# nrontsis/PILCO

Measured on AMD Instinct MI355X. Metric: moment-matching rollouts/sec (N=1000,D=10,E=10,H=40), higher is better.
Workload: dtype f64; 1 GPU; BASELINE configs[1]: N=1000 D=10 E=10 H=40 full rollout + reward, control_dim=0 (D==E read literally), ExponentialReward(W=I,t=0), factorisation cached (R-fwd); one step = one host-synchronised pilco_rollout call (what PILCO.predict makes) with its result downloaded; parallelism=pairs1, exchange=none (one rank)

## Files before the change

pilco_amd/csrc/glue_device.h:

```cpp
#pragma once
#include "mm_device.h"
#include "link_predicates.h"

namespace pilco {

struct GlueLds {
    double* mx;
    double* sx;
    double* mu;
    double* su;
    double* cxu;
    double* t1;
    double* t2;
    double* s1;
    double* jm;
    double* js;
    double* seg;
    double* mp;
    double* misc;
    double* pol;
    double* xm;
    double* xs;
    int nm;
    int o_sx, o_s1, o_js, o_seg, o_mp, o_misc;
};

__host__ __device__ __forceinline__ void glue_lds_carve(const GlueArgs& g, double* sm, GlueLds& L) {
    const int E = g.E, D = g.D;
    const int nm = E > D ? E : D;
    int seg_n = (g.flags & (GF_PACK | GF_ASSEMBLE)) ? g.wk.SEG * ((g.flags & GF_PACK) ? 1 : g.wk.nranks) : 0;
    if (g.flags & GF_RBF_POST) seg_n = g.pwk.SEG;
    L.mx = sm;
    L.sx = L.mx + nm;
    L.mu = L.sx + nm * nm;
    L.su = L.mu + nm;
    L.cxu = L.su + nm * nm;
    L.t1 = L.cxu + nm * nm;
    L.t2 = L.t1 + nm * nm;
    L.s1 = L.t2 + nm * nm;
    L.jm = L.s1 + nm * nm;
    L.js = L.jm + nm;
    L.misc = L.js + nm * nm;
    L.seg = L.misc + 256;
    L.mp = L.seg + seg_n;
    {
        const int mp_n = (g.flags & GF_RBF_POST) ? g.pwk.EL * g.pwk.NCHM * (1 + E) : ((g.flags & GF_PACK) ? g.wk.EL * g.wk.NCHM * (1 + D) : 0);
        const int rew_n = (int)reward_lds_doubles(E);
        const int tail = seg_n + mp_n;
        L.pol = L.seg + (tail > rew_n ? tail : rew_n);
    }
    L.xm = nullptr;
    L.xs = nullptr;
    L.nm = nm;
    L.o_sx = nm;
    L.o_s1 = 2 * nm + 5 * nm * nm;
    L.o_js = 3 * nm + 6 * nm * nm;
    L.o_seg = 3 * nm + 7 * nm * nm + 256;
    L.o_misc = 3 * nm + 7 * nm * nm;
    L.o_mp = L.o_seg + seg_n;
}

struct LoadSeg {
    int dst;
    const double* src;
    int n;
};
template <int NSEG, int MAXV>
__device__ __forceinline__ void multi_load(double* lds, const LoadSeg (&sg)[NSEG]) {
    int off[NSEG + 1];
    off[0] = 0;
#pragma unroll
    for (int i = 0; i < NSEG; ++i) off[i + 1] = off[i] + sg[i].n;
    const int total = off[NSEG];
    const int nthr = (int)blockDim.x;
    for (int base = 0; base < total; base += MAXV * nthr) {
        double v[MAXV];
#pragma unroll
        for (int k = 0; k < MAXV; ++k) {
            const int e = base + k * nthr + (int)threadIdx.x;
            v[k] = 0.0;
            if (e < total) {
#pragma unroll
                for (int i = 0; i < NSEG; ++i)
                    if (e >= off[i] && e < off[i + 1]) v[k] = sg[i].src[e - off[i]];
            }
        }
#pragma unroll
        for (int k = 0; k < MAXV; ++k) {
            const int e = base + k * nthr + (int)threadIdx.x;
            if (e < total) {
#pragma unroll
                for (int i = 0; i < NSEG; ++i)
                    if (e >= off[i] && e < off[i + 1]) lds[sg[i].dst + (e - off[i])] = v[k];
            }
        }
    }
}

__device__ __forceinline__ void squash_inplace(const GlueLds& L, int U, const double* maxact, double* cdiag, double* sc_alt = nullptr, bool eval_only = false) {
    const int t = threadIdx.x;
    const int nm = L.nm;
    double* sc = sc_alt ? sc_alt : L.t1;
    const int cap = sc_alt ? 5 * (U * U + U) : PILCO_SQUASH_ROUND_CAP(nm);
    const int nitems = U * U + U;
    double newS[4] = {0.0, 0.0, 0.0, 0.0};
    double newM = 0.0, newC = 0.0;
    for (int i0 = 0; i0 < 5 * nitems; i0 += cap) {
        const int n = (5 * nitems - i0) < cap ? (5 * nitems - i0) : cap;
        {
            const int w = t >> 6, f = w % 3, nw = (int)blockDim.x >> 6;
            const int nwf = (nw - f + 2) / 3;
            const int qa = i0 / 5, qb = (i0 + n) / 5;
            const int nc = (U * U > qa) ? ((U * U < qb ? U * U : qb) - qa) : 0, nu = (qb - qa) - nc;
            const int cnt = (f == 0) ? 3 * nc + nu : (f == 1) ? 2 * nc + nu : nu;
            for (int e = (w / 3) * 64 + (t & 63); e < cnt; e += nwf * 64) {
                int q, j;
                if (f == 0) {
                    if (e < 3 * nc) { q = qa + e / 3; j = e - 3 * (e / 3); } else { q = qa + nc + (e - 3 * nc); j = 0; }
                } else if (f == 1) {
                    if (e < 2 * nc) { q = qa + (e >> 1); j = 3 + (e & 1); } else { q = qa + nc + (e - 2 * nc); j = 1; }
                } else {
                    q = qa + nc + e; j = 2;
                }
                double arg;
                if (q < U * U) {
                    int v;
                    const int u = idiv_s(q, U, v);
                    const double lq = -(L.su[u * U + u] + L.su[v * U + v]) / 2.0;
                    const double suv = L.su[q];
                    arg = (j == 0) ? lq : (j == 1) ? lq + suv : (j == 2) ? lq - suv : (j == 3) ? L.mu[u] - L.mu[v] : L.mu[u] + L.mu[v];
                } else {
                    const int u = q - U * U;
                    arg = (j == 0) ? -L.su[u * U + u] / 2.0 : L.mu[u];
                }
                double val;
                if (f == 0) val = exp(arg);
                else if (f == 1) val = cos(arg);
                else val = sin(arg);
                sc[5 * (q - qa) + j] = val;
            }
        }
        __syncthreads();
        if (eval_only) return;
        const int q0 = i0 / 5, q1 = (i0 + n) / 5;
#pragma unroll
        for (int k = 0; k < 4; ++k) {
            const int e = t + k * (int)blockDim.x;
            if (e < U * U && e >= q0 && e < q1) {
                int v;
// ... 71 lines not shown
}

__device__ __forceinline__ void write_joint_lin_squash(const GlueArgs& g, const GlueLds& L, bool writer, const double* sq, const double* maxact) {
    const int E = g.E, U = g.U, D = g.D, t = threadIdx.x;
    double* s1_dst = g.s1_out ? g.s1_out : g.s1;
    auto cdiag_of = [&](int u) { const double* r = sq + 5 * (U * U + u); return (maxact ? maxact[u] : 1.0) * r[0] * r[1]; };
    if (t < D) {
        double v;
        if (t < E) v = L.mx[t];
        else {
            const int u = t - E;
            const double* r = sq + 5 * (U * U + u);
            v = (maxact ? maxact[u] : 1.0) * r[0] * r[2];
        }
        L.jm[t] = v;
        if (L.xm) L.xm[t] = v;
        if (writer) {
            g.wk.in_m[t] = v;
            if (g.tape) g.tape[(long)g.step * (D + D * D + E * D + E + E * E + D * E) + t] = v;
        }
    }
    for (int e = t; e < D * D; e += blockDim.x) {
        int c;
        const int r = idiv_s(e, D, c);
        double v;
        if (r < E && c < E) v = L.sx[r * E + c];
        else if (r < E) v = L.t1[(c - E) * E + r] * cdiag_of(c - E);
        else if (c < E) v = L.t1[(r - E) * E + c] * cdiag_of(r - E);
        else {
            const int u = r - E, v2 = c - E;
            const double* q = sq + 5 * (u * U + v2);
            const double val = (q[1] - q[0]) * q[3] - (q[2] - q[0]) * q[4];
            v = (maxact ? maxact[u] * maxact[v2] : 1.0) * val / 2.0;
        }
        L.js[e] = v;
        if (L.xs) L.xs[e] = v;
        if (writer) {
            g.wk.in_s[e] = v;
            if (r < E) s1_dst[r * D + c] = v;
            if (g.tape) {
                double* rec = g.tape + (long)g.step * (D + D * D + E * D + E + E * E + D * E);
                rec[D + e] = v;
                if (r < E) rec[D + D * D + r * D + c] = v;
            }
        }
    }
    __syncthreads();
}

struct PackPre {
    double v[16];
    double isdet;
};
__device__ __forceinline__ void mm_pack_issue(const MMWork& wk, int base, PackPre& pp) {
    const int t = threadIdx.x;
    const int k = base + (t >> 2), gq = t & 3;
    pp.isdet = 0.0;
#pragma unroll
    for (int u = 0; u < 16; ++u) pp.v[u] = 0.0;
    if (t >= 256 || k >= wk.PL) return;
    pp.isdet = wk.pair_isdet[k];
    if (wk.sk_waves > 0) {
        const int qw = wk.sk_maxw >> 2;
        const double* src = wk.sk_part + (long)(gq * qw) * wk.sk_pls + k;
#pragma unroll
        for (int u = 0; u < 16; ++u)
            if (u < qw) pp.v[u] = src[(long)u * wk.sk_pls];
    } else {
        const double* part = wk.pair_part + (long)k * wk.NT * 2;
        const int q0 = (int)((long)wk.NT * gq / 4), q1 = (int)((long)wk.NT * (gq + 1) / 4);
#pragma unroll
        for (int u = 0; u < 8; ++u)
            if (q0 + u < q1) {
                pp.v[2 * u] = part[2 * (q0 + u)];
                pp.v[2 * u + 1] = part[2 * (q0 + u) + 1];
            }
    }
}
__device__ __forceinline__ void mm_pack_sum(const MMWork& wk, int base, const PackPre& pp, double& s0, double& s1) {
    const int t = threadIdx.x;
    const int k = base + (t >> 2), gq = t & 3;
    s0 = 0.0;
    s1 = 0.0;
    if (t >= 256 || k >= wk.PL) return;
    if (wk.sk_waves > 0) {
#pragma unroll
        for (int u = 0; u < 16; ++u) s0 += pp.v[u];
        const int qw = wk.sk_maxw >> 2;
        const double* src = wk.sk_part + (long)(gq * qw) * wk.sk_pls + k;
        for (int u0 = 16; u0 < qw; u0 += 8) {
            double w8[8];
#pragma unroll
            for (int u = 0; u < 8; ++u) w8[u] = src[(long)min(u0 + u, qw - 1) * wk.sk_pls];
#pragma unroll
            for (int u = 0; u < 8; ++u) s0 += (u0 + u < qw) ? w8[u] : 0.0;
        }
    } else {
        const double* part = wk.pair_part + (long)k * wk.NT * 2;
        const int q0 = (int)((long)wk.NT * gq / 4), q1 = (int)((long)wk.NT * (gq + 1) / 4);
#pragma unroll
        for (int u = 0; u < 8; ++u)
            if (q0 + u < q1) {
                s0 += pp.v[2 * u];
                s1 += pp.v[2 * u + 1];
            }
        for (int q = q0 + 8; q < q1; ++q) {
            s0 += part[2 * q];
            s1 += part[2 * q + 1];
        }
    }
}

__device__ __forceinline__ void mm_pack(const MMWork& wk, int D, int E, const GlueLds& L, PackPre& pp, bool writer) {
    const int t = threadIdx.x;
    double* seg = wk.gath + (long)wk.rank * wk.SEG;
    for (int base = 0; base < wk.PL; base += 64) {
        const int k = base + (t >> 2), gq = t & 3;
        if (base > 0) mm_pack_issue(wk, base, pp);
        double s0, s1;
        mm_pack_sum(wk, base, pp, s0, s1);
        s0 += __shfl_xor(s0, 1);
        s1 += __shfl_xor(s1, 1);
        s0 += __shfl_xor(s0, 2);
        s1 += __shfl_xor(s1, 2);
        if (t < 256 && k < wk.PL && gq == 0) {
            const bool diag = k * wk.nranks + wk.rank < E;
            const double v = (diag ? (s0 - s1) : s0) * pp.isdet;
            if (writer) seg[k] = v;
            L.seg[k] = v;
        }
    }
    const int W1 = 1 + D;
    for (int e = t; e < wk.EL * W1; e += blockDim.x) {
        int idx;
        const int o = idiv_s(e, W1, idx);
        double sum = 0.0;
        _Pragma("unroll 8") for (int ch = 0; ch < wk.NCHM; ++ch) sum += L.mp[(o * wk.NCHM + ch) * W1 + idx];
        if (writer) seg[wk.OUTOFF + e] = sum;
        L.seg[wk.OUTOFF + e] = sum;
    }
    __syncthreads();
}

__device__ __forceinline__ void mm_assemble(const MMWork& wk, const double* src, const double* var, int D, int E, double* oM,
                            double* oS, double* oV, bool writer) {
    const int t = threadIdx.x;
    for (int a = t; a < E; a += blockDim.x) {
        const double v = src[(a % wk.nranks) * wk.SEG + wk.OUTOFF + (a / wk.nranks) * (1 + D)];
        oM[a] = v;
        if (writer) wk.out_M[a] = v;
    }
    for (int e = t; e < D * E; e += blockDim.x) {
        int a;
        const int d = idiv_s(e, E, a);
        const double v = src[(a % wk.nranks) * wk.SEG + wk.OUTOFF + (a / wk.nranks) * (1 + D) + 1 + d];
        oV[e] = v;
        if (writer) wk.out_V[e] = v;
    }
    __syncthreads();
    for (int e = t; e < E * E; e += blockDim.x) {
        int b;
        const int a = idiv_s(e, E, b);
        const int hi = a > b ? a : b, lo = a > b ? b : a;
        const int kk = pair_order_index(E, hi, lo);
        double v = src[(kk % wk.nranks) * wk.SEG + kk / wk.nranks];
        if (a == b) v += var[a];
        v = fma(-oM[a], oM[b], v);
        oS[e] = v;
        if (writer) wk.out_S[e] = v;
    }
    __syncthreads();
// ... 227 lines not shown
                        for (int c = 0; c < E; ++c) y = fma(Q[r * E + c], xrow[c], y);
                        quad = fma(xrow[r], y, quad);
                    }
                    vv[ii] = kk + quad;
                } else {
                    double* ytmp = pt + bf * (2 * E + 2) + ii * 16;
                    for (int r = 0; r < E; ++r) {
                        double y = 0.0;
                        for (int c = 0; c < E; ++c) y = fma(Q[r * E + c], xrow[c], y);
                        quad = fma(xrow[r], y, quad);
                        ytmp[r] = 2.0 * y;
                    }
                    for (int r = 0; r < E; ++r) xrow[r] = ytmp[r];
                    uv[ii] = kk + quad;
                }
            }
        }
        __syncthreads();
        if (do2 && t <= E) red[t] = ((red[t] + red[(E + 2) + t]) + red[2 * (E + 2) + t]) + red[3 * (E + 2) + t];
        if (do3 && t < 256) {
            double acc = 0.0;
            for (int idx = t; idx < bf * bf; idx += 256) {
                int j;
                const int i = idiv_s(idx, bf, j);
                double e = uv[i] + vv[j];
                for (int d = 0; d < E; ++d) e = fma(pv[i * E + d], wv[j * E + d], e);
                acc = fma(bet[a * bf + i] * bet[b * bf + j], exp(e), acc);
            }
            const double sacc = wave_sum_lane63(acc);
            if (lane == 63) red3[w] = sacc;
        }
        __syncthreads();
        if (do2) {
            const double cu = var[u] / sqrt(det[u]);
            if (t == 0) L.mu[u] = cu * red[0];
            if (t < E) {
                double acc = 0.0;
                for (int kq = 0; kq < E; ++kq) acc = fma(Tm[(u * E + t) * E + kq], red[1 + kq], acc);
                L.cxu[t * U + u] = cu * acc;
            }
        }
        if (do3 && t == 0) {
            const double N = (red3[0] + red3[1]) + (red3[2] + red3[3]);
            double v = N / sqrt(det[U + pq]);
            if (a == b) v += var[a];
            v = fma(-L.mu[a], L.mu[b], v);
            L.su[a * U + b] = v;
            L.su[b * U + a] = v;
        }
        __syncthreads();
    }
}

template <int PK = -1, bool SR = false>
__device__ __forceinline__ void glue_body(const GlueArgs& g, const GlueLds& L, bool writer) {
    const int E = g.E, D = g.D, U = g.U, t = threadIdx.x;
    int mp_n = (g.flags & GF_PACK) ? g.wk.EL * g.wk.NCHM * (1 + D) : 0;
    int seg_n = (g.flags & (GF_PACK | GF_ASSEMBLE)) ? g.wk.SEG * ((g.flags & GF_PACK) ? 1 : g.wk.nranks) : 0;
    if (g.flags & GF_RBF_POST) {
        mp_n = g.pwk.EL * g.pwk.NCHM * (1 + E);
        seg_n = g.pwk.SEG;
    }
    const bool dbg0 = (t == 0) && writer;
    const int dbo = g.dbg_off ? g.dbg_off : ((g.step == 0) ? 16 : 0);
    DBG_STAMP(g.wk, 8 + dbo, dbg0);
    PackPre pp;
    if ((g.flags & GF_PACK) && !MM_ABL(g.wk, 16)) mm_pack_issue(g.wk, 0, pp);
    const bool xq_in = !SR && g.xq && (g.flags & GF_ASSEMBLE) && !(g.flags & GF_PACK);
    if constexpr (!SR)
        if (xq_in) xq_wait(g);
    {
        const bool need_state = (g.flags & (GF_PROPAGATE | GF_TRAJ | GF_POLICY | GF_RBF_PRE)) != 0;
        const bool lin = (g.flags & GF_POLICY) && g.pol_kind == PILCO_POLICY_LINEAR;
        const bool pol = (g.flags & GF_POLICY) && g.pol_kind != PILCO_POLICY_NONE;
        const LoadSeg sg[8] = {
            {0, g.m_x, need_state ? E : 0},
            {L.o_sx, g.s_x, need_state ? E * E : 0},
            {L.o_s1, g.s1, (g.flags & GF_PROPAGATE) ? E * D : 0},
            {L.o_mp, (g.flags & GF_RBF_POST) ? g.pwk.mean_part : g.wk.mean_part, mp_n},
            {L.o_seg, g.wk.gath, ((g.flags & GF_ASSEMBLE) && !(g.flags & GF_PACK) && !xq_in) ? seg_n : 0},
            {L.o_js, g.W, lin ? U * E : 0},
            {L.o_misc + 128, g.b, lin ? U : 0},
            {L.o_misc + 160, g.maxact, (pol && g.maxact) ? U : 0},
        };
        RbfPre rpre;
        const bool rbf_in = (PK < 0 || PK == 2) && (g.flags & GF_POLICY) && g.pol_kind == PILCO_POLICY_RBF && g.pol_inline;
        if constexpr (PK < 0 || PK == 2)
            if (rbf_in) rbf_policy_preload_round(g, L, 0, rpre, true, false);
        multi_load<8, 4>(L.mx, sg);
        if constexpr (PK < 0 || PK == 2)
            if (rbf_in) rbf_policy_preload_rest(g, L, rpre);
        if constexpr (!SR)
            if (xq_in) xq_load_segments(g, L.seg);
    }
    __syncthreads();

    DBG_STAMP(g.wk, 9 + dbo, dbg0);
    if ((g.flags & GF_PACK) && !MM_ABL(g.wk, 16)) mm_pack(g.wk, D, E, L, pp, writer);
    if constexpr (!SR)
        if ((g.flags & GF_PACK) && g.xq_peers && writer) xq_push(g, L.seg);
    DBG_STAMP(g.wk, 10 + dbo, dbg0);
    const bool fast = (g.flags & (GF_PACK | GF_ASSEMBLE | GF_PROPAGATE)) == (GF_PACK | GF_ASSEMBLE | GF_PROPAGATE) && g.wk.nranks == 1;
    const bool joint_is_state = (PK == 0) && fast && (g.flags & GF_POLICY) && !g.act_out && U == 0;
    if (fast) {
        const double* seg = L.seg;
        const int W1 = 1 + D, OO = g.wk.OUTOFF;
        for (int e = t; e < E * E; e += blockDim.x) {
            int c;
            const int r = idiv_s(e, E, c);
            const int hi = r > c ? r : c, lo = r > c ? c : r;
            double v = seg[pair_order_index(E, hi, lo)];
            if (r == c) v += g.var[r];
            v = fma(-seg[OO + r * W1], seg[OO + c * W1], v);
            L.su[e] = v;
            double acc = 0.0;
            _Pragma("unroll 8") for (int k = 0; k < D; ++k) acc = fma(L.s1[r * D + k], seg[OO + c * W1 + 1 + k], acc);
            L.t1[e] = acc;
        }
        if (t < E) L.mu[t] = seg[OO + t * W1];
        if (writer && g.tape) {
            for (int e = t; e < D * E; e += blockDim.x) {
                int a_;
                const int d_ = idiv_s(e, E, a_);
                L.cxu[e] = seg[OO + a_ * W1 + 1 + d_];
            }
        }
        __syncthreads();
        if (writer && g.tape && g.step >= 1) {
            double* rec = g.tape + (long)(g.step - 1) * (D + D * D + E * D + E + E * E + D * E) + D + D * D + E * D;
            if (t < E) rec[t] = L.mu[t];
            for (int e = t; e < E * E; e += blockDim.x) rec[E + e] = L.su[e];
            for (int e = t; e < D * E; e += blockDim.x) rec[E + E * E + e] = L.cxu[e];
        }
        double* s1_dst = g.s1_out ? g.s1_out : g.s1;
        double* trec = g.tape ? g.tape + (long)g.step * (D + D * D + E * D + E + E * E + D * E) : nullptr;
        for (int e = t; e < E * E; e += blockDim.x) {
            int c;
            const int r = idiv_s(e, E, c);
            const double v = ((L.su[e] + L.sx[e]) + L.t1[e]) + L.t1[c * E + r];
            L.sx[e] = v;
            if (writer) g.s_out[e] = v;
            if (joint_is_state) {
                L.js[e] = v;
                if (L.xs) L.xs[e] = v;
                if (writer) {
                    g.wk.in_s[e] = v;
                    s1_dst[e] = v;
                    if (trec) {
                        trec[D + e] = v;
                        trec[D + D * D + e] = v;
                    }
// ... 25 lines not shown
        }
    }
    DBG_STAMP(g.wk, 11 + dbo, dbg0);
    if (!SR && !fast && (g.flags & GF_PROPAGATE)) {
        for (int e = t; e < E * E; e += blockDim.x) {
            int c;
            const int r = idiv_s(e, E, c);
            double acc = 0.0;
            _Pragma("unroll 8") for (int k = 0; k < D; ++k) acc = fma(L.s1[r * D + k], L.cxu[k * E + c], acc);
            L.t1[e] = acc;
        }
        __syncthreads();
        for (int e = t; e < E * E; e += blockDim.x) {
            int c;
            const int r = idiv_s(e, E, c);
            const double v = ((L.su[e] + L.sx[e]) + L.t1[e]) + L.t1[c * E + r];
            L.t2[e] = v;
            if (writer) g.s_out[e] = v;
        }
        if (t < E) {
            const double v = L.mu[t] + L.mx[t];
            L.misc[96 + t] = v;
            if (writer) g.m_out[t] = v;
        }
        __syncthreads();
        for (int e = t; e < E * E; e += blockDim.x) L.sx[e] = L.t2[e];
        if (t < E) L.mx[t] = L.misc[96 + t];
        __syncthreads();
    }
    DBG_STAMP(g.wk, 12 + dbo, dbg0);
    if (writer && (g.flags & GF_TRAJ) && g.traj) {
        double* dst = g.traj + (long)g.step * (E + E * E);
        if (t < E) dst[t] = L.mx[t];
        for (int e = t; e < E * E; e += blockDim.x) dst[E + e] = L.sx[e];
    }
    if (writer && (g.flags & GF_RBF_PRE)) {
        if (t < E) g.pwk.in_m[t] = L.mx[t];
        for (int e = t; e < E * E; e += blockDim.x) g.pwk.in_s[e] = L.sx[e];
    }
    if (g.flags & GF_POLICY) {
        const double* jcd = nullptr;
        bool lin_fused = false;
        if (PK != 0 && PK != 3 && g.pol_kind == PILCO_POLICY_RBF) {
            bool done = false;
            if constexpr (PK < 0 || PK == 2) {
                if (g.pol_inline) {
                    rbf_policy_inline(g, L);
                    done = true;
                }
            }
            if constexpr (PK < 0 || PK == 1) {
                if (!done) {
                    PackPre pq;
                    mm_pack_issue(g.pwk, 0, pq);
                    mm_pack(g.pwk, E, U, L, pq, writer);
                    mm_assemble(g.pwk, L.seg, g.pvar, E, U, L.mu, L.su, L.cxu, writer);
                }
            }
            if (t < U) L.su[t * U + t] -= g.pvar[t] - 1e-6;
            __syncthreads();
            if (g.squash) {
                double* cdiag = L.misc + 1;
                squash_inplace(L, U, g.maxact ? L.misc + 160 : nullptr, cdiag);
                if (g.act_out) {
                    for (int e = t; e < E * U; e += blockDim.x) L.cxu[e] *= cdiag[e % U];
                    __syncthreads();
                } else {
                    jcd = cdiag;
                }
            }
        }
        if ((PK < 0 || PK == 3) && g.pol_kind == PILCO_POLICY_LINEAR) {
            if (t < U) {
                double acc = L.misc[128 + t];
                _Pragma("unroll 8") for (int k = 0; k < E; ++k) acc = fma(L.js[t * E + k], L.mx[k], acc);
                L.mu[t] = acc;
            }
            for (int e = t; e < U * E; e += blockDim.x) {
                int c;
                const int u = idiv_s(e, E, c);
                double acc = 0.0;
                _Pragma("unroll 8") for (int k = 0; k < E; ++k) acc = fma(L.js[u * E + k], L.sx[k * E + c], acc);
                L.t1[e] = acc;
                L.cxu[c * U + u] = L.js[e];
            }
            __syncthreads();
            for (int e = t; e < U * U; e += blockDim.x) {
                int v;
                const int u = idiv_s(e, U, v);
                double acc = 0.0;
                _Pragma("unroll 8") for (int k = 0; k < E; ++k) acc = fma(L.t1[u * E + k], L.js[v * E + k], acc);
                L.su[e] = acc;
            }
            __syncthreads();
#ifdef LINK_STAMPS
            DBG_STAMP(g.wk, 36, dbg0);
#endif
            if (g.squash) {
                double* cdiag = L.misc + 1;
                lin_fused = !g.act_out && !joint_is_state && PILCO_SQUASH_LIN_FUSED_FITS(U, L.nm);
                squash_inplace(L, U, g.maxact ? L.misc + 160 : nullptr, cdiag, lin_fused ? L.t2 : nullptr, lin_fused);
                if (g.act_out) {
                    for (int e = t; e < E * U; e += blockDim.x) L.cxu[e] *= cdiag[e % U];
                    __syncthreads();
                } else {
                    jcd = cdiag;
                }
            }
#ifdef LINK_STAMPS
            DBG_STAMP(g.wk, 37, dbg0);
#endif
        }
        if (g.act_out) {
            if (writer) {
                if (t < U) g.act_out[t] = L.mu[t];
                for (int e = t; e < U * U; e += blockDim.x) g.act_out[U + e] = L.su[e];
                for (int e = t; e < E * U; e += blockDim.x) g.act_out[U + U * U + e] = L.cxu[e];
            }
        } else if (!joint_is_state) {
            if (lin_fused) write_joint_lin_squash(g, L, writer, L.t2, g.maxact ? L.misc + 160 : nullptr);
            else write_joint(g, L, writer, jcd);
        }
    }
    DBG_STAMP(g.wk, 13 + dbo, dbg0);
}

}
```

pilco_amd/csrc/prep_device.h:

```cpp
#pragma once
#include "glue_device.h"
#include "pair_device.h"

namespace pilco {

constexpr int PREP_TAB_DOUBLES = FEXP_TN + 8;
__host__ __device__ constexpr size_t prep_region_doubles(int DT) {
    const size_t stage = 256 * (size_t)(DT + 1),
                 ops = mm_kp(DT) <= 16 ? (size_t)mm_kp(DT) * (64 + 256) + 256 + (DT <= 14 ? 16 * 64 + 256 + 8 * 64 : 0) : 0;
    const size_t pair_blk = (size_t)4 * DT + 2 * (size_t)DT * DT + 4 + (stage > ops ? stage : ops);
    const size_t mean_blk = (size_t)2 * DT + 2 * (size_t)DT * DT + 4 + 9 * (size_t)(DT + 1) + 2 * (size_t)DT + 512 * (size_t)(DT + 2);
    return pair_blk > mean_blk ? pair_blk : mean_blk;
}
struct PrepHeadLds {
    int gd;
    size_t bytes;
};
inline PrepHeadLds prep_head_lds(int DT, size_t link_doubles, int reward_E) {
    const size_t work = prep_region_doubles(DT) + PREP_TAB_DOUBLES;
    const size_t rw = reward_E > 0 ? (size_t)reward_E + (size_t)reward_E * reward_E + reward_lds_doubles(reward_E) : 0;
    const size_t gd = (link_doubles + 1) & ~(size_t)1;
    return {(int)gd, sizeof(double) * ((work > rw ? work : rw) + gd)};
}

template <int DT>
__device__ __forceinline__ void prep_wt_constants(const MMModel& md, const MMWork& wk, int pl, double* sm) {
    const int R = wt_rows_per_pair(wk), t = threadIdx.x;
    if (wt_rows_dealt(wk) && t < R && pl * R + t < md.E * md.D) {
        const double l = md.ls[pl * R + t];
        sm[3 * DT + 2 * DT * DT + 4 + t] = 1.0 / (l * l);
    }
}

template <int DT, bool FUSED, int NTHR, bool PRE = false>
__device__ __forceinline__ void prep_mean_block(const MMModel& md, const MMWork& wk, int al, int chm, double* sm,
                                                const double* jm, const double* js,
                                                const double la_t, const double var_a) {
    const int D = md.D, npad = md.npad;
    const int t = threadIdx.x, lane = t & 63;
    const int w = __builtin_amdgcn_readfirstlane(t >> 6);
    const bool act = (NTHR == 512) || t < 512;
    const int a = al * wk.nranks + wk.rank;
    double* s_m = sm;
    double* s_ia = s_m + DT;
    double* s_s = s_ia + DT;
    double* s_T = s_s + DT * DT;
    double* s_sc = s_T + DT * DT;
    double* red = s_sc + 4;
    double* colbuf = red + 9 * (DT + 1);
    double* zst = colbuf + 2 * DT;
    double* bst = zst + 512 * (DT + 1);
    constexpr int LDZ = DT | 1;
    if constexpr (!PRE) {
        if (t < DT) {
            s_m[t] = (t < D) ? (FUSED ? jm[t] : wk.in_m[t]) : 0.0;
            s_ia[t] = (t < D) ? 1.0 / la_t : 0.0;
        }
        for (int e = t; e < D * D; e += 512) s_s[e] = FUSED ? js[e] : wk.in_s[e];
        for (int e = t; e < DT * DT; e += 512) s_T[e] = 0.0;
        __syncthreads();
    }
    const bool dbgm = (t == 0 && al == 0 && chm == 0);
    DBG_STAMP(wk, 40, dbgm);
    const int rpc = npad >> __builtin_ctz(wk.NCHM);
    const int i_begin = chm * rpc, i_end = i_begin + rpc;
    if (w == 0) {
        double col[DT];
        const int c = lane;
        const bool in_s = c < D;
        const double ic = in_s ? s_ia[c] : 0.0;
        double sv[DT], ir[DT];
#pragma unroll
        for (int r = 0; r < DT; ++r) {
            sv[r] = s_s[(in_s && r < D) ? r * D + c : 0];
            ir[r] = s_ia[r];
        }
#pragma unroll
        for (int r = 0; r < DT; ++r) {
            const double sval = (in_s && r < D) ? sv[r] : 0.0;
            col[r] = c < DT ? fma(sval, ir[r] * ic, (r == c) ? 1.0 : 0.0) : ((c < 2 * DT && c - DT == r) ? 1.0 : 0.0);
        }
// ... 561 lines not shown
```

pilco_amd/csrc/prep_kernel.h:

```cpp
#pragma once
#include "prep_device.h"

namespace pilco {

#ifndef PREP_SPARE_FIRST
#define PREP_SPARE_FIRST 1
#endif
#ifndef PREP_PRE
#define PREP_PRE 1
#endif

template <int DT, bool FUSED, int PK = 0, bool SR = true, bool OCC2 = false>
__global__ __launch_bounds__(512, OCC2 ? 4 : 2) void k_mm_prep(MMModel md, MMWork wk, PrepReward pr, GlueArgs g, int glue_doubles) {
    extern __shared__ __attribute__((aligned(16))) double sm_all[];
    kernarg_warm<(int)(sizeof(MMModel) + sizeof(MMWork) + sizeof(PrepReward) + sizeof(GlueArgs)) + 8 + 64>();
    GlueLds L;
    glue_lds_carve(g, sm_all, L);
    const int bxi = PREP_SPARE_FIRST ? (int)((blockIdx.x + (unsigned)wk.PL) % gridDim.x) : (int)blockIdx.x;
    const bool spare_wg = bxi >= wk.PL;
    const int spare_idx = (bxi - wk.PL) * (int)gridDim.y + (int)blockIdx.y;
    const bool mean_wg = spare_wg && spare_idx < wk.EL * wk.NCHM;
    int a = 0, b = 0;
    if (!spare_wg) local_pair_ab(wk, md.E, bxi, a, b);
    else if (mean_wg) a = b = (spare_idx >> __builtin_ctz(wk.NCHM)) * wk.nranks + wk.rank;
    double pre_la = 1.0, pre_lb = 1.0, pre_var = 1.0;
    if (!spare_wg || mean_wg) {
        if ((int)threadIdx.x < md.D) {
            pre_la = md.ls[a * md.D + (int)threadIdx.x];
            pre_lb = md.ls[b * md.D + (int)threadIdx.x];
        }
        pre_var = mean_wg ? md.var[a] : md.lvar[(threadIdx.x >> 8) ? b : a];
    }
    if (FUSED && SR && PK != 1 && wk.fuse_pair && !spare_wg) {
        double* tabL = sm_all + glue_doubles + prep_region_doubles(DT);
        for (int e = threadIdx.x; e < FEXP_TN; e += 512) tabL[e] = fexp_table_unbias(wk.exp_tab[e], e);
    }
    constexpr bool PRE = FUSED && PK != 1 && (PREP_PRE != 0);
    if constexpr (PRE) {
        double* sm = sm_all + glue_doubles;
        const int t = threadIdx.x, D = md.D;
        if (!spare_wg) {
            if (t < DT) {
                if (t >= D) sm[t] = 0.0;
                sm[DT + t] = (t < D) ? 1.0 / (pre_la * pre_la) : 0.0;
                sm[2 * DT + t] = (t < D) ? 1.0 / (pre_lb * pre_lb) : 0.0;
            }
            for (int e = t; e < DT * DT; e += 512) sm[3 * DT + DT * DT + e] = 0.0;
            prep_wt_constants<DT>(md, wk, bxi, sm);
            L.xm = sm;
            L.xs = sm + 3 * DT;
        } else if (mean_wg) {
            if (t < DT) {
                if (t >= D) sm[t] = 0.0;
                sm[DT + t] = (t < D) ? 1.0 / pre_la : 0.0;
            }
            for (int e = t; e < DT * DT; e += 512) sm[2 * DT + DT * DT + e] = 0.0;
            L.xm = sm;
            L.xs = sm + 2 * DT;
        }
    }
    if (FUSED) glue_body<PK, SR>(g, L, bxi == 0 && blockIdx.y == 0);
    prep_work<DT, FUSED, 512, FUSED && SR && PK != 1, PRE>(md, wk, pr, g, L, sm_all, glue_doubles, bxi, (int)blockIdx.y, (int)gridDim.x, (int)gridDim.y, a, b, pre_la,
                              pre_lb, pre_var);
}

struct PrepLaunch {
    hipStream_t st;
    dim3 grid;
    PrepHeadLds lds;
    bool fused, multi;
    int pk;
    const MMModel* md;
    const MMWork* wk;
    const PrepReward* r;
    const GlueArgs* ga;
};

template <int DT>
void launch_prep_dt(const PrepLaunch& a) {
    const hipStream_t st = a.st;
    const dim3 grid = a.grid;
    const size_t lds = a.lds.bytes;
    const int gd = a.lds.gd, pk = a.pk;
    const bool fused = a.fused, multi = a.multi;
    const MMModel& md = *a.md;
    const MMWork& wk = *a.wk;
    const PrepReward& r = *a.r;
    const GlueArgs& ga = *a.ga;
#define PREP2(DT_, F_, PK_, SR_, O_) launch_lds<k_mm_prep<DT_, F_, PK_, SR_, O_>>(grid, dim3(512), lds, st, md, wk, r, ga, gd)
#define PREP1(DT_, F_, PK_, SR_)                                                                           \
    do {                                                                                                   \
        if constexpr (F_ && SR_ && (PK_ == 2 || PK_ == 3) && DT_ <= 8) {                                   \
            if (wk.share_cu) PREP2(DT_, F_, PK_, SR_, true);                                               \
            else PREP2(DT_, F_, PK_, SR_, false);                                                          \
        } else {                                                                                           \
            PREP2(DT_, F_, PK_, SR_, false);                                                               \
        }                                                                                                  \
    } while (0)
#define PREP(DT_)                                              \
    do {                                                       \
        if (!fused) PREP1(DT_, false, 0, true);                \
        else if (multi) {    \
            if (pk == 0) PREP1(DT_, true, 0, false);           \
            else if (pk == 3) PREP1(DT_, true, 3, false);      \
            else PREP1(DT_, true, 2, false);                   \
        } else if (pk == 0) PREP1(DT_, true, 0, true);         \
        else if (pk == 3) PREP1(DT_, true, 3, true);           \
        else if (pk == 1) PREP1(DT_, true, 1, true);           \
        else PREP1(DT_, true, 2, true);                        \
    } while (0)
    PREP(DT);
#undef PREP
#undef PREP1
#undef PREP2
}

// ... 12 lines not shown
```

Baseline: 431.7 rollouts/s.

## Issue glue and constant global loads early in fused prep kernel head

Splits the glue body into a request phase, which issues the first round of global loads into registers, and a finish phase, which stores them to LDS. The fused prep kernel now issues these requests at entry, before the pair-index and constant setup, so the load latencies overlap. Constants such as lengthscales, weights and the exp table are also loaded unconditionally up front and written to LDS later, inside the glue finish step. The cost is more register pressure and some extra unconditional loads. Optional wall-clock stamps behind a macro are added for measuring the kernel head.

New measurement: 435.2 rollouts/s, median of 6. Within noise of the previous version (+0.8%).

```diff
diff --git a/pilco_amd/csrc/glue_device.h b/pilco_amd/csrc/glue_device.h
--- a/pilco_amd/csrc/glue_device.h
+++ b/pilco_amd/csrc/glue_device.h
@@ -23,6 +23,10 @@
     double* xs;
     int nm;
     int o_sx, o_s1, o_js, o_seg, o_mp, o_misc;
+#ifdef HEAD_START_STAMP
+    unsigned long long hs_entry, hs_warm;
+    int hs_slot;
+#endif
 };
 
 __host__ __device__ __forceinline__ void glue_lds_carve(const GlueArgs& g, double* sm, GlueLds& L) {
@@ -51,6 +55,10 @@
     }
     L.xm = nullptr;
     L.xs = nullptr;
+#ifdef HEAD_START_STAMP
+    L.hs_entry = L.hs_warm = 0;
+    L.hs_slot = -1;
+#endif
     L.nm = nm;
     L.o_sx = nm;
     L.o_s1 = 2 * nm + 5 * nm * nm;
@@ -65,8 +73,71 @@
     const double* src;
     int n;
 };
+template <int NSEG, int MAXV, int NTHR = 0>
+__device__ __forceinline__ void multi_load_request(const LoadSeg (&sg)[NSEG], const int (&off)[NSEG + 1], const double* first, int base, double (&v)[MAXV],
+                                                   int (&d)[MAXV]) {
+    const int total = off[NSEG], nthr = NTHR ? NTHR : (int)blockDim.x;
+    const int w0 = __builtin_amdgcn_readfirstlane((int)threadIdx.x) & ~63;
+#pragma unroll
+    for (int k = 0; k < MAXV; ++k) {
+        const int e = base + k * nthr + (int)threadIdx.x;
+        v[k] = 0.0;
+        d[k] = -1;
+        if (base + k * nthr + w0 < total) {
+            const double* src = first;
+            int dst = -1;
+#pragma unroll
+            for (int i = 0; i < NSEG; ++i)
+                if (e >= off[i]) {
+                    src = sg[i].src + (e - off[i]);
+                    dst = sg[i].dst + (e - off[i]);
+                }
+            if (e >= total) {
+                src = first;
+                dst = -1;
+            }
+            v[k] = *src;
+            d[k] = dst;
+        }
+    }
+}
+template <int MAXV>
+__device__ __forceinline__ void multi_load_store(double* lds, const double (&v)[MAXV], const int (&d)[MAXV]) {
+#pragma unroll
+    for (int k = 0; k < MAXV; ++k)
+        if (d[k] >= 0) lds[d[k]] = v[k];
+}
+template <int NSEG>
+__device__ __forceinline__ const double* multi_load_offsets(const LoadSeg (&sg)[NSEG], int (&off)[NSEG + 1]) {
+    off[0] = 0;
+#pragma unroll
+    for (int i = 0; i < NSEG; ++i) off[i + 1] = off[i] + sg[i].n;
+    const double* first = nullptr;
+#pragma unroll
+    for (int i = NSEG - 1; i >= 0; --i)
+        if (sg[i].n > 0) first = sg[i].src;
+    return first;
+}
+template <int NSEG, int MAXV, int NTHR = 0>
+__device__ __forceinline__ void multi_load_first(const LoadSeg (&sg)[NSEG], double (&v)[MAXV], int (&d)[MAXV]) {
+    int off[NSEG + 1];
+    const double* first = multi_load_offsets<NSEG>(sg, off);
+    multi_load_request<NSEG, MAXV, NTHR>(sg, off, first, 0, v, d);
+}
+template <int NSEG, int MAXV, int NTHR = 0>
+__device__ __forceinline__ void multi_load_rest(double* lds, const LoadSeg (&sg)[NSEG]) {
+    int off[NSEG + 1];
+    const double* first = multi_load_offsets<NSEG>(sg, off);
+    const int total = off[NSEG], nthr = NTHR ? NTHR : (int)blockDim.x;
+    for (int base = MAXV * nthr; base < total; base += MAXV * nthr) {
+        double v[MAXV];
+        int d[MAXV];
+        multi_load_request<NSEG, MAXV, NTHR>(sg, off, first, base, v, d);
+        multi_load_store<MAXV>(lds, v, d);
+    }
+}
 template <int NSEG, int MAXV>
-__device__ __forceinline__ void multi_load(double* lds, const LoadSeg (&sg)[NSEG]) {
+__device__ __forceinline__ void multi_load_by_segment(double* lds, const LoadSeg (&sg)[NSEG]) {
     int off[NSEG + 1];
     off[0] = 0;
 #pragma unroll
@@ -95,6 +166,14 @@
             }
         }
     }
+}
+template <int NSEG, int MAXV>
+__device__ __forceinline__ void multi_load(double* lds, const LoadSeg (&sg)[NSEG]) {
+    double v[MAXV];
+    int d[MAXV];
+    multi_load_first<NSEG, MAXV>(sg, v, d);
+    multi_load_store<MAXV>(lds, v, d);
+    multi_load_rest<NSEG, MAXV>(lds, sg);
 }
 
 __device__ __forceinline__ void squash_inplace(const GlueLds& L, int U, const double* maxact, double* cdiag, double* sc_alt = nullptr, bool eval_only = false) {
@@ -272,6 +351,7 @@
     double v[16];
     double isdet;
 };
+template <bool NEWF = true>
 __device__ __forceinline__ void mm_pack_issue(const MMWork& wk, int base, PackPre& pp) {
     const int t = threadIdx.x;
     const int k = base + (t >> 2), gq = t & 3;
@@ -279,7 +359,7 @@
 #pragma unroll
     for (int u = 0; u < 16; ++u) pp.v[u] = 0.0;
     if (t >= 256 || k >= wk.PL) return;
-    pp.isdet = wk.pair_isdet[k];
+    if constexpr (!NEWF) pp.isdet = wk.pair_isdet[k];
     if (wk.sk_waves > 0) {
         const int qw = wk.sk_maxw >> 2;
         const double* src = wk.sk_part + (long)(gq * qw) * wk.sk_pls + k;
@@ -296,6 +376,7 @@
                 pp.v[2 * u + 1] = part[2 * (q0 + u) + 1];
             }
     }
+    if constexpr (NEWF) pp.isdet = wk.pair_isdet[k];
 }
 __device__ __forceinline__ void mm_pack_sum(const MMWork& wk, int base, const PackPre& pp, double& s0, double& s1) {
     const int t = threadIdx.x;
@@ -331,12 +412,13 @@
     }
 }
 
+template <bool NEWF = true>
 __device__ __forceinline__ void mm_pack(const MMWork& wk, int D, int E, const GlueLds& L, PackPre& pp, bool writer) {
     const int t = threadIdx.x;
     double* seg = wk.gath + (long)wk.rank * wk.SEG;
     for (int base = 0; base < wk.PL; base += 64) {
         const int k = base + (t >> 2), gq = t & 3;
-        if (base > 0) mm_pack_issue(wk, base, pp);
+        if (base > 0) mm_pack_issue<NEWF>(wk, base, pp);
         double s0, s1;
         mm_pack_sum(wk, base, pp, s0, s1);
         s0 += __shfl_xor(s0, 1);
@@ -670,51 +752,97 @@
     }
 }
 
-template <int PK = -1, bool SR = false>
-__device__ __forceinline__ void glue_body(const GlueArgs& g, const GlueLds& L, bool writer) {
-    const int E = g.E, D = g.D, U = g.U, t = threadIdx.x;
-    int mp_n = (g.flags & GF_PACK) ? g.wk.EL * g.wk.NCHM * (1 + D) : 0;
-    int seg_n = (g.flags & (GF_PACK | GF_ASSEMBLE)) ? g.wk.SEG * ((g.flags & GF_PACK) ? 1 : g.wk.nranks) : 0;
+struct GlueNoMid {
+    __device__ __forceinline__ void operator()() const {}
+};
+struct GlueReq {
+    PackPre pp;
+    double v[4];
+    int d[4];
+    RbfPre rpre;
+};
+__device__ __forceinline__ void glue_sizes(const GlueArgs& g, int& mp_n, int& seg_n) {
+    mp_n = (g.flags & GF_PACK) ? g.wk.EL * g.wk.NCHM * (1 + g.D) : 0;
+    seg_n = (g.flags & (GF_PACK | GF_ASSEMBLE)) ? g.wk.SEG * ((g.flags & GF_PACK) ? 1 : g.wk.nranks) : 0;
     if (g.flags & GF_RBF_POST) {
-        mp_n = g.pwk.EL * g.pwk.NCHM * (1 + E);
+        mp_n = g.pwk.EL * g.pwk.NCHM * (1 + g.E);
         seg_n = g.pwk.SEG;
     }
+}
+template <bool SR>
+__device__ __forceinline__ bool glue_xq_in(const GlueArgs& g) {
+    return !SR && g.xq && (g.flags & GF_ASSEMBLE) && !(g.flags & GF_PACK);
+}
+template <int PK>
+__device__ __forceinline__ bool glue_rbf_in(const GlueArgs& g) {
+    return (PK < 0 || PK == 2) && (g.flags & GF_POLICY) && g.pol_kind == PILCO_POLICY_RBF && g.pol_inline;
+}
+__device__ __forceinline__ void glue_segments(const GlueArgs& g, const GlueLds& L, bool xq_in, LoadSeg (&sg)[8]) {
+    const int E = g.E, D = g.D, U = g.U;
+    int mp_n, seg_n;
+    glue_sizes(g, mp_n, seg_n);
+    const bool need_state = (g.flags & (GF_PROPAGATE | GF_TRAJ | GF_POLICY | GF_RBF_PRE)) != 0;
+    const bool lin = (g.flags & GF_POLICY) && g.pol_kind == PILCO_POLICY_LINEAR;
+    const bool pol = (g.flags & GF_POLICY) && g.pol_kind != PILCO_POLICY_NONE;
+    sg[0] = LoadSeg{0, g.m_x, need_state ? E : 0};
+    sg[1] = LoadSeg{L.o_sx, g.s_x, need_state ? E * E : 0};
+    sg[2] = LoadSeg{L.o_s1, g.s1, (g.flags & GF_PROPAGATE) ? E * D : 0};
+    sg[3] = LoadSeg{L.o_mp, (g.flags & GF_RBF_POST) ? g.pwk.mean_part : g.wk.mean_part, mp_n};
+    sg[4] = LoadSeg{L.o_seg, g.wk.gath, ((g.flags & GF_ASSEMBLE) && !(g.flags & GF_PACK) && !xq_in) ? seg_n : 0};
+    sg[5] = LoadSeg{L.o_js, g.W, lin ? U * E : 0};
+    sg[6] = LoadSeg{L.o_misc + 128, g.b, lin ? U : 0};
+    sg[7] = LoadSeg{L.o_misc + 160, g.maxact, (pol && g.maxact) ? U : 0};
+}
+template <int PK = -1, bool SR = false, int NTHR = 0>
+__device__ __forceinline__ void glue_request(const GlueArgs& g, const GlueLds& L, bool writer, GlueReq& q) {
+    const int t = threadIdx.x;
     const bool dbg0 = (t == 0) && writer;
     const int dbo = g.dbg_off ? g.dbg_off : ((g.step == 0) ? 16 : 0);
     DBG_STAMP(g.wk, 8 + dbo, dbg0);
-    PackPre pp;
-    if ((g.flags & GF_PACK) && !MM_ABL(g.wk, 16)) mm_pack_issue(g.wk, 0, pp);
-    const bool xq_in = !SR && g.xq && (g.flags & GF_ASSEMBLE) && !(g.flags & GF_PACK);
+    if ((g.flags & GF_PACK) && !MM_ABL(g.wk, 16)) mm_pack_issue<true>(g.wk, 0, q.pp);
+#ifdef HEAD_START_STAMP
+    if (g.wk.dbg && t == 0 && L.hs_slot >= 0) {
+        const unsigned long long now = wall_clock64();
+        g.wk.dbg[L.hs_slot ? 54 : 14] = L.hs_entry;
+        g.wk.dbg[L.hs_slot ? 55 : 15] = L.hs_warm;
+        g.wk.dbg[L.hs_slot ? 62 : 19] = now;
+    }
+#endif
+    const bool xq_in = glue_xq_in<SR>(g);
     if constexpr (!SR)
         if (xq_in) xq_wait(g);
-    {
-        const bool need_state = (g.flags & (GF_PROPAGATE | GF_TRAJ | GF_POLICY | GF_RBF_PRE)) != 0;
-        const bool lin = (g.flags & GF_POLICY) && g.pol_kind == PILCO_POLICY_LINEAR;
-        const bool pol = (g.flags & GF_POLICY) && g.pol_kind != PILCO_POLICY_NONE;
-        const LoadSeg sg[8] = {
-            {0, g.m_x, need_state ? E : 0},
-            {L.o_sx, g.s_x, need_state ? E * E : 0},
-            {L.o_s1, g.s1, (g.flags & GF_PROPAGATE) ? E * D : 0},
-            {L.o_mp, (g.flags & GF_RBF_POST) ? g.pwk.mean_part : g.wk.mean_part, mp_n},
-            {L.o_seg, g.wk.gath, ((g.flags & GF_ASSEMBLE) && !(g.flags & GF_PACK) && !xq_in) ? seg_n : 0},
-            {L.o_js, g.W, lin ? U * E : 0},
-            {L.o_misc + 128, g.b, lin ? U : 0},
-            {L.o_misc + 160, g.maxact, (pol && g.maxact) ? U : 0},
-        };
-        RbfPre rpre;
-        const bool rbf_in = (PK < 0 || PK == 2) && (g.flags & GF_POLICY) && g.pol_kind == PILCO_POLICY_RBF && g.pol_inline;
-        if constexpr (PK < 0 || PK == 2)
-            if (rbf_in) rbf_policy_preload_round(g, L, 0, rpre, true, false);
-        multi_load<8, 4>(L.mx, sg);
-        if constexpr (PK < 0 || PK == 2)
-            if (rbf_in) rbf_policy_preload_rest(g, L, rpre);
-        if constexpr (!SR)
-            if (xq_in) xq_load_segments(g, L.seg);
-    }
+    if constexpr (PK < 0 || PK == 2)
+        if (glue_rbf_in<PK>(g)) rbf_policy_preload_round(g, L, 0, q.rpre, true, false);
+    LoadSeg sg[8];
+    glue_segments(g, L, xq_in, sg);
+    multi_load_first<8, 4, NTHR>(sg, q.v, q.d);
+}
+
+template <int PK, bool SR, bool NEWF>
+__device__ __forceinline__ void glue_tail(const GlueArgs& g, const GlueLds& L, bool writer, PackPre& pp);
+template <int PK = -1, bool SR = false, int NTHR = 0, class Mid = GlueNoMid>
+__device__ __forceinline__ void glue_finish(const GlueArgs& g, const GlueLds& L, bool writer, GlueReq& q, const Mid& mid = Mid()) {
+    const bool xq_in = glue_xq_in<SR>(g);
+    mid();
+    LoadSeg sg[8];
+    glue_segments(g, L, xq_in, sg);
+    multi_load_store<4>(L.mx, q.v, q.d);
+    multi_load_rest<8, 4, NTHR>(L.mx, sg);
+    if constexpr (PK < 0 || PK == 2)
+        if (glue_rbf_in<PK>(g)) rbf_policy_preload_rest(g, L, q.rpre);
+    if constexpr (!SR)
+        if (xq_in) xq_load_segments(g, L.seg);
+    glue_tail<PK, SR, true>(g, L, writer, q.pp);
+}
+template <int PK, bool SR, bool NEWF>
+__device__ __forceinline__ void glue_tail(const GlueArgs& g, const GlueLds& L, bool writer, PackPre& pp) {
+    const int E = g.E, D = g.D, U = g.U, t = threadIdx.x;
+    const bool dbg0 = (t == 0) && writer;
+    const int dbo = g.dbg_off ? g.dbg_off : ((g.step == 0) ? 16 : 0);
     __syncthreads();
 
     DBG_STAMP(g.wk, 9 + dbo, dbg0);
-    if ((g.flags & GF_PACK) && !MM_ABL(g.wk, 16)) mm_pack(g.wk, D, E, L, pp, writer);
+    if ((g.flags & GF_PACK) && !MM_ABL(g.wk, 16)) mm_pack<NEWF>(g.wk, D, E, L, pp, writer);
     if constexpr (!SR)
         if ((g.flags & GF_PACK) && g.xq_peers && writer) xq_push(g, L.seg);
     DBG_STAMP(g.wk, 10 + dbo, dbg0);
@@ -846,8 +974,8 @@
             if constexpr (PK < 0 || PK == 1) {
                 if (!done) {
                     PackPre pq;
-                    mm_pack_issue(g.pwk, 0, pq);
-                    mm_pack(g.pwk, E, U, L, pq, writer);
+                    mm_pack_issue<NEWF>(g.pwk, 0, pq);
+                    mm_pack<NEWF>(g.pwk, E, U, L, pq, writer);
                     mm_assemble(g.pwk, L.seg, g.pvar, E, U, L.mu, L.su, L.cxu, writer);
                 }
             }
@@ -918,5 +1046,54 @@
     }
     DBG_STAMP(g.wk, 13 + dbo, dbg0);
 }
-
-}
+template <int PK = -1, bool SR = false, bool NEWF = true>
+__device__ __forceinline__ void glue_body(const GlueArgs& g, const GlueLds& L, bool writer) {
+    if constexpr (NEWF) {
+        GlueReq q;
+        glue_request<PK, SR>(g, L, writer, q);
+        glue_finish<PK, SR>(g, L, writer, q);
+    } else {
+        const int E = g.E, D = g.D, U = g.U, t = threadIdx.x;
+        int mp_n = (g.flags & GF_PACK) ? g.wk.EL * g.wk.NCHM * (1 + D) : 0;
+        int seg_n = (g.flags & (GF_PACK | GF_ASSEMBLE)) ? g.wk.SEG * ((g.flags & GF_PACK) ? 1 : g.wk.nranks) : 0;
+        if (g.flags & GF_RBF_POST) {
+            mp_n = g.pwk.EL * g.pwk.NCHM * (1 + E);
+            seg_n = g.pwk.SEG;
+        }
+        const bool dbg0 = (t == 0) && writer;
+        const int dbo = g.dbg_off ? g.dbg_off : ((g.step == 0) ? 16 : 0);
+        DBG_STAMP(g.wk, 8 + dbo, dbg0);
+        PackPre pp;
+        if ((g.flags & GF_PACK) && !MM_ABL(g.wk, 16)) mm_pack_issue<false>(g.wk, 0, pp);
+        const bool xq_in = !SR && g.xq && (g.flags & GF_ASSEMBLE) && !(g.flags & GF_PACK);
+        if constexpr (!SR)
+            if (xq_in) xq_wait(g);
+        {
+            const bool need_state = (g.flags & (GF_PROPAGATE | GF_TRAJ | GF_POLICY | GF_RBF_PRE)) != 0;
+            const bool lin = (g.flags & GF_POLICY) && g.pol_kind == PILCO_POLICY_LINEAR;
+            const bool pol = (g.flags & GF_POLICY) && g.pol_kind != PILCO_POLICY_NONE;
+            const LoadSeg sg[8] = {
+                {0, g.m_x, need_state ? E : 0},
+                {L.o_sx, g.s_x, need_state ? E * E : 0},
+                {L.o_s1, g.s1, (g.flags & GF_PROPAGATE) ? E * D : 0},
+                {L.o_mp, (g.flags & GF_RBF_POST) ? g.pwk.mean_part : g.wk.mean_part, mp_n},
+                {L.o_seg, g.wk.gath, ((g.flags & GF_ASSEMBLE) && !(g.flags & GF_PACK) && !xq_in) ? seg_n : 0},
+                {L.o_js, g.W, lin ? U * E : 0},
+                {L.o_misc + 128, g.b, lin ? U : 0},
+                {L.o_misc + 160, g.maxact, (pol && g.maxact) ? U : 0},
+            };
+            RbfPre rpre;
+            const bool rbf_in = (PK < 0 || PK == 2) && (g.flags & GF_POLICY) && g.pol_kind == PILCO_POLICY_RBF && g.pol_inline;
+            if constexpr (PK < 0 || PK == 2)
+                if (rbf_in) rbf_policy_preload_round(g, L, 0, rpre, true, false);
+            multi_load_by_segment<8, 4>(L.mx, sg);
+            if constexpr (PK < 0 || PK == 2)
+                if (rbf_in) rbf_policy_preload_rest(g, L, rpre);
+            if constexpr (!SR)
+                if (xq_in) xq_load_segments(g, L.seg);
+        }
+        glue_tail<PK, SR, false>(g, L, writer, pp);
+    }
+}
+
+}
diff --git a/pilco_amd/csrc/prep_device.h b/pilco_amd/csrc/prep_device.h
--- a/pilco_amd/csrc/prep_device.h
+++ b/pilco_amd/csrc/prep_device.h
@@ -23,10 +23,21 @@
     return {(int)gd, sizeof(double) * ((work > rw ? work : rw) + gd)};
 }
 
+__device__ __forceinline__ bool prep_wt_has(const MMModel& md, const MMWork& wk, int pl) {
+    const int R = wt_rows_per_pair(wk), t = threadIdx.x;
+    return wt_rows_dealt(wk) && t < R && pl * R + t < md.E * md.D;
+}
+__device__ __forceinline__ double prep_wt_request(const MMModel& md, const MMWork& wk, int pl, bool pair_wg) {
+    return md.ls[(pair_wg && prep_wt_has(md, wk, pl)) ? pl * wt_rows_per_pair(wk) + (int)threadIdx.x : 0];
+}
+template <int DT>
+__device__ __forceinline__ void prep_wt_commit(const MMModel& md, const MMWork& wk, int pl, double* sm, double l) {
+    if (prep_wt_has(md, wk, pl)) sm[3 * DT + 2 * DT * DT + 4 + (int)threadIdx.x] = 1.0 / (l * l);
+}
 template <int DT>
 __device__ __forceinline__ void prep_wt_constants(const MMModel& md, const MMWork& wk, int pl, double* sm) {
     const int R = wt_rows_per_pair(wk), t = threadIdx.x;
-    if (wt_rows_dealt(wk) && t < R && pl * R + t < md.E * md.D) {
+    if (prep_wt_has(md, wk, pl)) {
         const double l = md.ls[pl * R + t];
         sm[3 * DT + 2 * DT * DT + 4 + t] = 1.0 / (l * l);
     }
diff --git a/pilco_amd/csrc/prep_kernel.h b/pilco_amd/csrc/prep_kernel.h
--- a/pilco_amd/csrc/prep_kernel.h
+++ b/pilco_amd/csrc/prep_kernel.h
@@ -9,59 +9,173 @@
 #ifndef PREP_PRE
 #define PREP_PRE 1
 #endif
-
-template <int DT, bool FUSED, int PK = 0, bool SR = true, bool OCC2 = false>
-__global__ __launch_bounds__(512, OCC2 ? 4 : 2) void k_mm_prep(MMModel md, MMWork wk, PrepReward pr, GlueArgs g, int glue_doubles) {
-    extern __shared__ __attribute__((aligned(16))) double sm_all[];
-    kernarg_warm<(int)(sizeof(MMModel) + sizeof(MMWork) + sizeof(PrepReward) + sizeof(GlueArgs)) + 8 + 64>();
+#ifndef PREP_CONST_LATE
+#define PREP_CONST_LATE 1
+#endif
+#ifndef PREP_REQ_EARLY
+#define PREP_REQ_EARLY 1
+#endif
+
+template <int DT, int PK>
+__device__ __forceinline__ void prep_head_requests_first(const MMModel& md, const MMWork& wk, const PrepReward& pr, const GlueArgs& g, int glue_doubles,
+                                                         double* sm_all, const unsigned long long (&hs)[2]) {
+    (void)hs;
     GlueLds L;
     glue_lds_carve(g, sm_all, L);
     const int bxi = PREP_SPARE_FIRST ? (int)((blockIdx.x + (unsigned)wk.PL) % gridDim.x) : (int)blockIdx.x;
     const bool spare_wg = bxi >= wk.PL;
+    constexpr bool FUSED = true, SR = true;
+    constexpr bool EARLY = PREP_REQ_EARLY != 0;
+    GlueReq rq;
+#ifdef HEAD_START_STAMP
+    L.hs_entry = hs[0];
+    L.hs_warm = hs[1];
+    L.hs_slot = (bxi == 0 && blockIdx.y == 0) ? 0 : (blockIdx.x == gridDim.x - 1 && blockIdx.y == gridDim.y - 1 && !spare_wg) ? 1 : -1;
+#endif
+    if constexpr (EARLY) glue_request<PK, SR, 512>(g, L, bxi == 0 && blockIdx.y == 0, rq);
     const int spare_idx = (bxi - wk.PL) * (int)gridDim.y + (int)blockIdx.y;
     const bool mean_wg = spare_wg && spare_idx < wk.EL * wk.NCHM;
     int a = 0, b = 0;
     if (!spare_wg) local_pair_ab(wk, md.E, bxi, a, b);
     else if (mean_wg) a = b = (spare_idx >> __builtin_ctz(wk.NCHM)) * wk.nranks + wk.rank;
+    constexpr bool PRE = FUSED && PK != 1 && (PREP_PRE != 0);
+    constexpr bool LATE = PRE && (PREP_CONST_LATE != 0);
     double pre_la = 1.0, pre_lb = 1.0, pre_var = 1.0;
-    if (!spare_wg || mean_wg) {
+    if constexpr (LATE) {
+        const int dd = (int)threadIdx.x < md.D ? (int)threadIdx.x : 0;
+        pre_la = md.ls[a * md.D + dd];
+        pre_lb = md.ls[b * md.D + dd];
+        pre_var = *(mean_wg ? md.var + a : md.lvar + ((threadIdx.x >> 8) ? b : a));
+    } else if (!spare_wg || mean_wg) {
         if ((int)threadIdx.x < md.D) {
             pre_la = md.ls[a * md.D + (int)threadIdx.x];
             pre_lb = md.ls[b * md.D + (int)threadIdx.x];
         }
         pre_var = mean_wg ? md.var[a] : md.lvar[(threadIdx.x >> 8) ? b : a];
     }
-    if (FUSED && SR && PK != 1 && wk.fuse_pair && !spare_wg) {
-        double* tabL = sm_all + glue_doubles + prep_region_doubles(DT);
+    static_assert(FEXP_TN <= 512, "one exp-table entry per thread");
+    const bool tab_on = FUSED && SR && PK != 1 && wk.fuse_pair && !spare_wg;
+    double* tabL = sm_all + glue_doubles + prep_region_doubles(DT);
+    double pre_wt = 1.0, pre_tab = 0.0;
+    if constexpr (LATE) {
+        pre_wt = prep_wt_request(md, wk, bxi, !spare_wg);
+        if (tab_on && (int)threadIdx.x < FEXP_TN) pre_tab = wk.exp_tab[threadIdx.x];
+    } else if (tab_on) {
         for (int e = threadIdx.x; e < FEXP_TN; e += 512) tabL[e] = fexp_table_unbias(wk.exp_tab[e], e);
     }
-    constexpr bool PRE = FUSED && PK != 1 && (PREP_PRE != 0);
     if constexpr (PRE) {
         double* sm = sm_all + glue_doubles;
-        const int t = threadIdx.x, D = md.D;
         if (!spare_wg) {
-            if (t < DT) {
-                if (t >= D) sm[t] = 0.0;
-                sm[DT + t] = (t < D) ? 1.0 / (pre_la * pre_la) : 0.0;
-                sm[2 * DT + t] = (t < D) ? 1.0 / (pre_lb * pre_lb) : 0.0;
-            }
-            for (int e = t; e < DT * DT; e += 512) sm[3 * DT + DT * DT + e] = 0.0;
-            prep_wt_constants<DT>(md, wk, bxi, sm);
             L.xm = sm;
             L.xs = sm + 3 * DT;
         } else if (mean_wg) {
-            if (t < DT) {
-                if (t >= D) sm[t] = 0.0;
-                sm[DT + t] = (t < D) ? 1.0 / pre_la : 0.0;
-            }
-            for (int e = t; e < DT * DT; e += 512) sm[2 * DT + DT * DT + e] = 0.0;
             L.xm = sm;
             L.xs = sm + 2 * DT;
         }
     }
-    if (FUSED) glue_body<PK, SR>(g, L, bxi == 0 && blockIdx.y == 0);
+    const auto consts = [&]() {
+        if constexpr (LATE) asm volatile("" : "+v"(pre_la), "+v"(pre_lb), "+v"(pre_wt), "+v"(pre_tab));
+        if constexpr (LATE)
+            if (tab_on && (int)threadIdx.x < FEXP_TN) tabL[threadIdx.x] = fexp_table_unbias(pre_tab, (int)threadIdx.x);
+        if constexpr (PRE) {
+            double* sm = sm_all + glue_doubles;
+            const int t = threadIdx.x, D = md.D;
+            if (!spare_wg) {
+                if (t < DT) {
+                    if (t >= D) sm[t] = 0.0;
+                    sm[DT + t] = (t < D) ? 1.0 / (pre_la * pre_la) : 0.0;
+                    sm[2 * DT + t] = (t < D) ? 1.0 / (pre_lb * pre_lb) : 0.0;
+                }
+                for (int e = t; e < DT * DT; e += 512) sm[3 * DT + DT * DT + e] = 0.0;
+                if constexpr (LATE) prep_wt_commit<DT>(md, wk, bxi, sm, pre_wt);
+                else prep_wt_constants<DT>(md, wk, bxi, sm);
+            } else if (mean_wg) {
+                if (t < DT) {
+                    if (t >= D) sm[t] = 0.0;
+                    sm[DT + t] = (t < D) ? 1.0 / pre_la : 0.0;
+                }
+                for (int e = t; e < DT * DT; e += 512) sm[2 * DT + DT * DT + e] = 0.0;
+            }
+        }
+    };
+    (void)consts;
+    if constexpr (FUSED) {
+        const bool writer = bxi == 0 && blockIdx.y == 0;
+        if constexpr (!LATE) consts();
+        if constexpr (!EARLY) glue_request<PK, SR, 512>(g, L, writer, rq);
+        if constexpr (LATE) glue_finish<PK, SR, 512>(g, L, writer, rq, consts);
+        else glue_finish<PK, SR, 512>(g, L, writer, rq);
+    }
     prep_work<DT, FUSED, 512, FUSED && SR && PK != 1, PRE>(md, wk, pr, g, L, sm_all, glue_doubles, bxi, (int)blockIdx.y, (int)gridDim.x, (int)gridDim.y, a, b, pre_la,
                               pre_lb, pre_var);
+}
+
+template <int DT, bool FUSED, int PK = 0, bool SR = true, bool OCC2 = false>
+__global__ __launch_bounds__(512, OCC2 ? 4 : 2) void k_mm_prep(MMModel md, MMWork wk, PrepReward pr, GlueArgs g, int glue_doubles) {
+    extern __shared__ __attribute__((aligned(16))) double sm_all[];
+#ifdef HEAD_START_STAMP
+    unsigned long long hs[2] = {wall_clock64(), 0};
+#else
+    const unsigned long long hs[2] = {0, 0};
+#endif
+    kernarg_warm<(int)(sizeof(MMModel) + sizeof(MMWork) + sizeof(PrepReward) + sizeof(GlueArgs)) + 8 + 64>();
+#ifdef HEAD_START_STAMP
+    hs[1] = wall_clock64();
+#endif
+    constexpr bool NEWF = FUSED && SR && !OCC2;
+    if constexpr (!NEWF) {
+        GlueLds L;
+        glue_lds_carve(g, sm_all, L);
+        const int bxi = PREP_SPARE_FIRST ? (int)((blockIdx.x + (unsigned)wk.PL) % gridDim.x) : (int)blockIdx.x;
+        const bool spare_wg = bxi >= wk.PL;
+        const int spare_idx = (bxi - wk.PL) * (int)gridDim.y + (int)blockIdx.y;
+        const bool mean_wg = spare_wg && spare_idx < wk.EL * wk.NCHM;
+        int a = 0, b = 0;
+        if (!spare_wg) local_pair_ab(wk, md.E, bxi, a, b);
+        else if (mean_wg) a = b = (spare_idx >> __builtin_ctz(wk.NCHM)) * wk.nranks + wk.rank;
+        double pre_la = 1.0, pre_lb = 1.0, pre_var = 1.0;
+        if (!spare_wg || mean_wg) {
+            if ((int)threadIdx.x < md.D) {
+                pre_la = md.ls[a * md.D + (int)threadIdx.x];
+                pre_lb = md.ls[b * md.D + (int)threadIdx.x];
+            }
+            pre_var = mean_wg ? md.var[a] : md.lvar[(threadIdx.x >> 8) ? b : a];
+        }
+        if (FUSED && SR && PK != 1 && wk.fuse_pair && !spare_wg) {
+            double* tabL = sm_all + glue_doubles + prep_region_doubles(DT);
+            for (int e = threadIdx.x; e < FEXP_TN; e += 512) tabL[e] = fexp_table_unbias(wk.exp_tab[e], e);
+        }
+        constexpr bool PRE = FUSED && PK != 1 && (PREP_PRE != 0);
+        if constexpr (PRE) {
+            double* sm = sm_all + glue_doubles;
+            const int t = threadIdx.x, D = md.D;
+            if (!spare_wg) {
+                if (t < DT) {
+                    if (t >= D) sm[t] = 0.0;
+                    sm[DT + t] = (t < D) ? 1.0 / (pre_la * pre_la) : 0.0;
+                    sm[2 * DT + t] = (t < D) ? 1.0 / (pre_lb * pre_lb) : 0.0;
+                }
+                for (int e = t; e < DT * DT; e += 512) sm[3 * DT + DT * DT + e] = 0.0;
+                prep_wt_constants<DT>(md, wk, bxi, sm);
+                L.xm = sm;
+                L.xs = sm + 3 * DT;
+            } else if (mean_wg) {
+                if (t < DT) {
+                    if (t >= D) sm[t] = 0.0;
+                    sm[DT + t] = (t < D) ? 1.0 / pre_la : 0.0;
+                }
+                for (int e = t; e < DT * DT; e += 512) sm[2 * DT + DT * DT + e] = 0.0;
+                L.xm = sm;
+                L.xs = sm + 2 * DT;
+            }
+        }
+        if (FUSED) glue_body<PK, SR, false>(g, L, bxi == 0 && blockIdx.y == 0);
+        prep_work<DT, FUSED, 512, FUSED && SR && PK != 1, PRE>(md, wk, pr, g, L, sm_all, glue_doubles, bxi, (int)blockIdx.y, (int)gridDim.x, (int)gridDim.y, a, b, pre_la,
+                                  pre_lb, pre_var);
+        return;
+    } else {
+        prep_head_requests_first<DT, PK>(md, wk, pr, g, glue_doubles, sm_all, hs);
+    }
 }
 
 struct PrepLaunch {
```
